# fgnt/padertorch

Measured on AMD Instinct MI355X. Metric: training frames/sec (PIT mask-est, 2-spk 8 kHz), higher is better.
Workload: dtype f32

## Files before the change

include/ptmi.h:

```cpp
#ifndef PTMI_H_
#define PTMI_H_

#include <stdint.h>

#ifdef __cplusplus
extern "C" {
#endif

#define PTMI_OK 0
#define PTMI_E_INVALID (-1)
#define PTMI_E_UNSUPPORTED (-2)

typedef void* ptmi_stream_t;

const char* ptmi_version(void);
const char* ptmi_error_string(int code);

typedef struct ptmi_stft_geom {
    int32_t size;
    int32_t shift;
    int32_t window_length;
    int32_t pad_left;
    int32_t pad_right;
    int32_t pad;
// ... 51 lines not shown


int ptmi_lstm_forward(float* gates, float* hy, float* c, const float* c0, const float* w_hh_pad, const int32_t* batch_sizes,
                      const int64_t* offsets, int32_t T, int32_t max_batch, int32_t H, int32_t KP,
                      int32_t ndir, ptmi_stream_t stream);

int ptmi_lstm_backward(const float* gates, const float* c, const float* c0, const float* dhy, const float* w_hh_t, float* dgates,
                       float* dc_state, const int32_t* batch_sizes, const int64_t* offsets, int32_t T,
                       int32_t max_batch, int32_t H, int32_t ndir, ptmi_stream_t stream);

int64_t ptmi_lstm_flags_elems(int32_t T, int32_t ndir, int32_t max_batch);
int64_t ptmi_lstm_scratch_elems(int32_t T, int32_t ndir, int32_t max_batch, int32_t H, int32_t backward);
int ptmi_lstm_weight_prep(const float* const* w_ih, const float* const* w_hh, const float* const* b_ih,
                          const float* const* b_hh, int32_t ndir, int32_t H, int32_t I, float* w_ih_cat, int32_t Ipad,
                          float* bias, float* w_pad, int32_t KP, float* w_t, uint32_t* amax, ptmi_stream_t stream);
int ptmi_lstm_set_error_sink(uint32_t* word);
int ptmi_lstm_split_enabled(void);
int32_t ptmi_lstm_handoff_cols(int32_t H, int32_t backward);
int32_t ptmi_lstm_backward_planes_ok(int32_t T, int32_t ndir, int32_t max_batch, int64_t rows, int32_t H);
int ptmi_lstm_forward_fills(int32_t T, int32_t ndir, int32_t max_batch, int32_t H);

int ptmi_lstm_forward_persistent(float* gates, float* hy, float* c, const float* c0, const float* w_hh_pad,
                                 const uint32_t* w_hh_amax, const int32_t* batch_sizes_dev, const int64_t* offsets_dev,
                                 const uint64_t* step_masks, uint32_t* flags, int32_t T, int32_t max_batch, int64_t rows,
                                 int32_t H, int32_t KP, int32_t ndir, int32_t prefilled, uint32_t* backward_scratch,
                                 ptmi_stream_t stream);

int ptmi_lstm_backward_persistent(const float* gates, const float* c, const float* c0, const float* dhy, const float* dc_n,
                                  const float* w_hh_t, float* dgates, uint16_t* dgates_t, const int32_t* batch_sizes_dev,
                                  const int64_t* offsets_dev, const uint64_t* step_masks, uint32_t* flags, float* dc_carry,
// ... 188 lines not shown
```

padertorch_amd/_lib.py:

```python
import ctypes
import os
import threading
from ctypes import c_char_p, c_double, c_float, c_int, c_int32, c_int64, c_void_p, POINTER
from pathlib import Path

import torch

_PKG = Path(__file__).resolve().parent
LIB_PATH = _PKG / 'libptmi.so'
if os.environ.get('PTMI_LIB'):
    LIB_PATH = Path(os.environ['PTMI_LIB'])


class StftGeom(ctypes.Structure):
    _fields_ = [('size', c_int32), ('shift', c_int32), ('window_length', c_int32),
                ('pad_left', c_int32), ('pad_right', c_int32), ('pad', c_int32)]


class NormGeom(ctypes.Structure):
    _fields_ = [('rank', c_int32), ('size', c_int64 * 5), ('stat_group_stride', c_int64 * 5),
                ('indep_stride', c_int64 * 5), ('batch_dim', c_int32), ('seq_dim', c_int32)]


_P = c_void_p
_G = POINTER(StftGeom)
_I64P = POINTER(c_int64)

SIGNATURES = {
    'ptmi_version': (c_char_p, []),
    'ptmi_error_string': (c_char_p, [c_int]),
    'ptmi_stft_num_frames': (c_int64, [_G, c_int64]),
    'ptmi_istft_num_samples': (c_int64, [_G, c_int64]),
    'ptmi_stft_forward': (c_int, [_P, c_int64, c_int64, c_int64, _P, _P, _P, _G, c_int64, c_int32,
                                  c_float, _P, _P]),
    'ptmi_istft_forward': (c_int, [_P, c_int64, c_int64, _P, _P, _P, _G, c_int32, c_float, c_int64,
                                   c_int64, c_int64, _P, _P]),
# ... 64 lines not shown
    'ptmi_dprnn_colsum': (c_int, [_P, c_int64, _P, _P, _P, c_int64, c_int32, _P]),
    'ptmi_dprnn_norm_residual_forward': (c_int, [_P, _P, _P, _P, _P, _P, _P, c_int64, c_int32, c_int32, c_int32, c_float, _P]),
    'ptmi_dprnn_norm_residual_backward': (c_int, [_P, _P, _P, _P, _P, _P, _P, _P, _P, c_int64, c_int32, c_int32, c_int32, _P]),
    'ptmi_dprnn_segment': (c_int, [_P, _I64P, _P, c_int64, c_int64, c_int32, c_int32, c_int32, c_int32, _P]),
    'ptmi_dprnn_overlap_add': (c_int, [_P, _I64P, _P, c_int64, c_int64, c_int32, c_int32, c_int32, c_int32, c_int32, _P]),
    'ptmi_lstm_forward': (c_int, [_P, _P, _P, _P, _P, _P, _P, c_int32, c_int32, c_int32, c_int32, c_int32, _P]),
    'ptmi_lstm_backward': (c_int, [_P, _P, _P, _P, _P, _P, _P, _P, _P, c_int32, c_int32, c_int32, c_int32, _P]),
    'ptmi_unit_norm_forward': (c_int, [_P, _P, _P, c_int64, c_int32, c_int32, c_float, c_void_p]),
    'ptmi_unit_norm_backward': (c_int, [_P, _P, _P, _P, c_int64, c_int32, c_int32, c_float, c_void_p]),
    'ptmi_lstm_flags_elems': (c_int64, [c_int32, c_int32, c_int32]),
    'ptmi_lstm_scratch_elems': (c_int64, [c_int32, c_int32, c_int32, c_int32, c_int32]),
    'ptmi_lstm_weight_prep': (c_int, [_P, _P, _P, _P, c_int32, c_int32, c_int32, _P, c_int32, _P, _P, c_int32, _P, _P, _P]),
    'ptmi_lstm_set_error_sink': (c_int, [_P]),
    'ptmi_lstm_split_enabled': (c_int, []),
    'ptmi_lstm_handoff_cols': (c_int32, [c_int32, c_int32]),
    'ptmi_lstm_forward_persistent': (c_int, [_P, _P, _P, _P, _P, _P, _P, _P, _P, _P, c_int32, c_int32, c_int64, c_int32, c_int32,
                                             c_int32, c_int32, _P, _P]),
    'ptmi_lstm_forward_fills': (c_int, [c_int32, c_int32, c_int32, c_int32]),
    'ptmi_lstm_backward_planes_ok': (c_int32, [c_int32, c_int32, c_int32, c_int64, c_int32]),
    'ptmi_lstm_backward_persistent': (c_int, [_P, _P, _P, _P, _P, _P, _P, _P, _P, _P, _P, _P, _P, c_int32, c_int32, c_int64, c_int32,
                                              c_int32, c_int32, c_int32, c_int32, _P]),
    'ptmi_absmax': (c_int, [_P, c_int64, c_int64, c_int64, _P, _P]),
    'ptmi_absmax_accumulate': (c_int, [_P, c_int64, c_int64, c_int64, _P, _P]),
    'ptmi_planes_elems': (c_int64, [c_int64, c_int64]),
    'ptmi_pack_planes_t': (c_int, [_P, c_int64, c_int64, c_int64, _P, _P, _P]),
    'ptmi_gemm_planes_workspace_elems': (c_int64, [c_int32, c_int32, c_int32, c_int32]),
    'ptmi_pack_planes_n': (c_int, [_P, c_int64, c_int64, c_int64, _P, _P, _P]),
    'ptmi_gemm_planes': (c_int, [_P, _P, _P, _P, _P, _P, c_int64, c_int32, c_int32, c_int32, c_int32, c_int32, c_int32, _P, _P]),
    'ptmi_gemm_planes_relu': (c_int, [_P, _P, _P, _P, _P, _P, c_int64, c_int32, c_int32, c_int32, c_int32, c_int32, _P, _P, c_int32, _P]),
    'ptmi_relu_backward_absmax': (c_int, [_P, _P, _P, c_int64, c_int64, c_int64, c_int64, c_int64, _P, c_int32, _P]),
# ... 184 lines not shown
```

padertorch_amd/csrc/gemm_planes.hip:

```cpp
#include <algorithm>

#include "common.h"

namespace ptmi {

typedef _Float16 h8 __attribute__((ext_vector_type(8)));
typedef __bf16 b8 __attribute__((ext_vector_type(8)));
typedef float f4 __attribute__((ext_vector_type(4)));

constexpr int PBM = 128, PBN = 128;
constexpr int FR = 64;

__device__ __forceinline__ float plane_scale(const unsigned* amax_bits) {
    if (!amax_bits) return 1.f;
    const unsigned e = (*amax_bits >> 23) & 0xffu;
    if (e == 0u || e == 0xffu) return 1.f;
    return __uint_as_float((unsigned)(127 + 13 + 127 - (int)e) << 23);
}

struct PlanesArgs {
    const uint4* A;
    const uint4* B;
    float* C;
    float* workspace;
    const unsigned* amax_a;
    const unsigned* amax_b;
    const float* bias;
    int M, N, KB;
    long long ldc;
    int accumulate;
    int kb_per_split;
    int tiles_m, tiles_n;
    float* C2 = nullptr;
// ... 503 lines not shown
        }
    } else {
        for (long long i = blockIdx.x * 256ll + threadIdx.x; i < n; i += (long long)gridDim.x * 256) {
            const long long r = i / cols, c = i - r * cols;
            m = max(m, __float_as_uint(x[r * ld + c]) & 0x7fffffffu);
        }
    }
#pragma unroll
    for (int o = 32; o > 0; o >>= 1) m = max(m, (unsigned)__shfl_xor((int)m, o));
    if ((threadIdx.x & 63) == 0) red[threadIdx.x >> 6] = m;
    __syncthreads();
    if (threadIdx.x == 0) {
        m = max(max(red[0], red[1]), max(red[2], red[3]));
        if (m >= 0x7f800000u) m = 0x7f7fffffu;
        atomicMax(out, m);
    }
}

template <bool BF16>
__device__ __forceinline__ void split_chunk(const float (&v)[8], uint4* hi_out, uint4* lo_out) {
    if (BF16) {
        b8 hi, lo;
#pragma unroll
        for (int e = 0; e < 8; ++e) {
            hi[e] = (__bf16)v[e];
            lo[e] = (__bf16)(v[e] - (float)hi[e]);
        }
        *hi_out = __builtin_bit_cast(uint4, hi);
        *lo_out = __builtin_bit_cast(uint4, lo);
    } else {
        h8 hi, lo;
#pragma unroll
        for (int e = 0; e < 8; ++e) {
            hi[e] = (_Float16)v[e];
            lo[e] = (_Float16)(v[e] - (float)hi[e]);
        }
        *hi_out = __builtin_bit_cast(uint4, hi);
        *lo_out = __builtin_bit_cast(uint4, lo);
    }
}

__global__ __launch_bounds__(256) void planes_reduce_kernel(const float* __restrict__ ws, int splits, float* __restrict__ C, long long ldc,
                                                            const float* __restrict__ bias, int M, int N, int accumulate,
                                                            float* __restrict__ C2 = nullptr, int m_split = 0, int relu = 0,
                                                            unsigned* __restrict__ amax_out = nullptr) {
    const long long total = (long long)M * N;
    unsigned mx = 0u;
    for (long long i = blockIdx.x * 256ll + threadIdx.x; i < total; i += (long long)gridDim.x * 256) {
        const int r = (int)(i / N), c = (int)(i - (long long)r * N);
        float sum = 0.f;
        for (int z = 0; z < splits; ++z) sum += ws[(long long)z * total + i];
        if (bias) sum += bias[c];
        if (relu) {
// ... 740 lines not shown
```

padertorch_amd/csrc/lstm_prep.hip:

```cpp
#include "common.h"

namespace ptmi {

constexpr int kIhPerWg = 16384;
constexpr int kStrip = 4;

struct PrepArgs {
    const float* w_ih[2];
    const float* w_hh[2];
    const float* b_ih[2];
    const float* b_hh[2];
    float* w_ih_cat;
    float* bias;
    float* w_pad;
    float* w_t;
    unsigned* amax;
    int ndir, G, I, Ipad, H, KP;
    int vec_ih;
    int blocks_ih;
    int tiles_g, strips_h;
};

__device__ __forceinline__ void publish_max(unsigned* word, float m, unsigned* red) {
    unsigned u = __float_as_uint(m);
// ... 136 lines not shown
    A.vec_ih = (I & 3) == 0 && Ipad == I;
    for (int d = 0; d < ndir; ++d) A.vec_ih = A.vec_ih && (reinterpret_cast<uintptr_t>(w_ih[d]) & 15) == 0;
    PTMI_RETURN_IF(reinterpret_cast<uintptr_t>(w_ih_cat) & 15, PTMI_E_INVALID);
    const long long total_ih = (long long)ndir * A.G * Ipad;
    A.blocks_ih = (int)((total_ih + kIhPerWg - 1) / kIhPerWg);
    A.tiles_g = (A.G + 31) / 32;
    A.strips_h = (KP + 32 * kStrip - 1) / (32 * kStrip);
    const int blocks_bias = (ndir * A.G + 255) / 256;
    hipStream_t st = static_cast<hipStream_t>(stream);
    hipError_t e = zero_words_async(amax, 2, st);
    if (e != hipSuccess) return (int)e;
    const unsigned grid = (unsigned)(A.blocks_ih + ndir * A.tiles_g * A.strips_h + blocks_bias);
    hipLaunchKernelGGL(lstm_weight_prep_kernel, dim3(grid), dim3(256), 0, st, A);
    return launch_status();
}
```

padertorch_amd/ops/gemm.py:

```python
import ctypes
import os
import threading
import weakref

import torch

from .. import _lib
from . import library

__all__ = ['mm', 'absmax', 'weight_absmax', 'UNIT_RANGE', 'PRODUCTS', 'ENABLED', 'usable']

ENABLED = True

PRODUCTS = 3

UNIT_RANGE = 'unit'

_WEIGHT_AMAX = {}


def _refs(params):
    return tuple(weakref.ref(p) for p in params)


# ... 100 lines not shown
    if len(cache) > limit:
        cache.clear()
    with torch.no_grad():
        v = make()
    cache[key] = (p._version, p.data_ptr(), v, _refs((p,)), _PREFETCHING[0])
    if form is not None:
        known = _KNOWN.get(id(p))
        if known is None or known[0]() is not p:
            if len(_KNOWN) > 256:
                _KNOWN.clear()
            known = _KNOWN[id(p)] = (weakref.ref(p), set())
        known[1].add(form)
    return v


def prefetch_known(device, everything=False):
    todo = []
    updated = _UPDATED.get(device)
    covered = updated[1] if updated is not None else {}
    for pid, (ref, forms) in list(_KNOWN.items()):
        q = ref()
        if q is None:
            del _KNOWN[pid]
        elif q.device == device and q.dim() == 2:
            e = covered.get(id(q))
            if everything or (e is not None and e[0]() is q and e[1] == q._version):
                todo.append((q, sorted(forms, key=str)))
    if not todo or _PREFETCHING[0] is not None:
        return
    ev = _PREFETCHING[0] = torch.cuda.Event()
    try:
        for q, forms in todo:
            for form in forms:
                if form == 'n':
                    weight_planes(q)
                elif form == 't':
                    weight_planes_t(q)
                else:
                    weight_planes_h(q, *form[1:])
    finally:
        _PREFETCHING[0] = None
        ev.record(torch.cuda.current_stream(device))


def weight_absmax(p):
    return _cached(_WEIGHT_AMAX, id(p), p, lambda: absmax(p.detach() if p.dim() == 2 else p.detach().reshape(-1, p.shape[-1])), 256)


def weights_absmax(params):
    params = tuple(params)
    if len(params) == 1:
        return weight_absmax(params[0])
    key = tuple(id(p) for p in params)
    sig = tuple((p._version, p.data_ptr()) for p in params)
    hit = _WEIGHT_AMAX.get(key)
    if hit is not None and hit[0] == sig and _same(hit[3], params):
        return hit[2]
# ... 187 lines not shown
```

padertorch_amd/ops/library.py:

```python
import ctypes
from typing import List, Optional, Tuple

import torch
from torch import Tensor

from .. import _lib

_LIBRARY = torch.library.Library('ptmi', 'DEF')


def _register(schema):
    name = schema.split('(', 1)[0].strip()

    def deco(fn):
        _LIBRARY.define(schema)
        _LIBRARY.impl(name, fn, 'CUDA')
        return getattr(torch.ops.ptmi, name)
    return deco


def _geom(g: List[int]):
    return _lib.StftGeom(*[int(v) for v in g])


# ... 539 lines not shown
@_register('lstm_weight_prep(Tensor[] w_ih, Tensor[] w_hh, Tensor[] b_ih, Tensor[] b_hh, int KP) -> '
           '(Tensor, Tensor, Tensor, Tensor, Tensor)')
def lstm_weight_prep(w_ih, w_hh, b_ih, b_hh, KP):
    ndir, (G, I), H = len(w_ih), w_ih[0].shape, w_hh[0].shape[1]
    dev = w_ih[0].device
    Ipad = (I + 3) // 4 * 4
    f32 = dict(dtype=torch.float32, device=dev)
    w_ih_cat, bias = torch.empty((ndir * G, Ipad), **f32), torch.empty(ndir * G, **f32)
    w_pad, w_t = torch.empty((ndir, G, KP), **f32), torch.empty((ndir, H, G), **f32)
    amax = torch.empty(2, dtype=torch.int32, device=dev)
    ptrs = [(ctypes.c_void_p * ndir)(*[t.data_ptr() for t in ts]) for ts in (w_ih, w_hh, b_ih, b_hh)]
    _lib.check(_lib.timed('lstm_weight_prep', _lib.load().ptmi_lstm_weight_prep, *ptrs, ndir, H, I, w_ih_cat.data_ptr(), Ipad,
                          bias.data_ptr(), w_pad.data_ptr(), KP, w_t.data_ptr(), amax.data_ptr(), _lib.stream(dev)),
               'ptmi_lstm_weight_prep')
    return w_ih_cat, bias, w_pad, w_t, amax


@_register('grad_norm(Tensor flat) -> Tensor')
def grad_norm(flat):
    lib = _lib.load()
    ws = torch.empty(int(lib.ptmi_grad_norm_workspace_elems()), dtype=torch.float64, device=flat.device)
    out = torch.empty((), dtype=torch.float32, device=flat.device)
    _lib.check(_lib.timed('grad_norm', lib.ptmi_grad_norm, flat.data_ptr(), flat.numel(), ws.data_ptr(), out.data_ptr(),
                          _lib.stream(flat.device)), 'ptmi_grad_norm')
    return out


@_register('adam_flat_(Tensor(a!) flat_grad, Tensor(b!) exp_avg, Tensor(c!) exp_avg_sq, Tensor segments, Tensor(d!)[] params, '
           'Tensor? norm, float max_norm, Tensor? found_inf, Tensor? finite, Tensor step, float lr, float beta1, float beta2, '
           'float eps, float weight_decay, bool zero_grad, Tensor? hyper=None) -> Tensor')
# ... 372 lines not shown
```

padertorch_amd/ops/lstm.py:

```python
import types

import torch
from torch.nn.utils.rnn import PackedSequence

from .. import _lib
from . import capture as _capture
from . import context as _context
from . import gemm as _gemm
from . import library
from . import lstm_forms as _forms
from . import watchdog as _watchdog
from . import wgrad as _wgrad
from .lstm_forms import begin_captured_step, end_captured_step
from .pack_meta import _PackMeta, _meta, pack_meta
from .watchdog import check_errors, error_count, error_word, errors_since_last_report, raise_timeout
from .wgrad import flush_pending as flush_pending_wgrad, gemm_keys_safe, sync_deferred, warm_side_stream, wgrad_key

__all__ = ['packed_lstm']


PERSISTENT = True
CHECK_PERSISTENT_ERRORS = False
DEFER_WGRAD = False
GRAD_READY_HOOK = None
# ... 578 lines not shown
    else:
        assert meta.rows == data.shape[0] and hx is None and not return_state and input_planes is None, 'row-slot batches: plain calls only'
        if not (PERSISTENT and _lib.load().ptmi_lstm_split_enabled()):
            raise NotImplementedError('row-slot batches need the persistent split recurrence kernels')
    sfx = ['', '_reverse'] if lstm.bidirectional else ['']
    ndir, H = len(sfx), lstm.hidden_size
    want_state = return_state or hx is not None
    if hx is not None:
        h_all, c_all = hx
        assert h_all.shape == c_all.shape == (lstm.num_layers * ndir, meta.max_batch, H), (h_all.shape, meta.max_batch)
    h_n, c_n = [], []
    h = data.contiguous()
    all_params = [tuple((getattr(lstm, f'weight_ih_l{layer}{s}'), getattr(lstm, f'weight_hh_l{layer}{s}'),
                         getattr(lstm, f'bias_ih_l{layer}{s}'), getattr(lstm, f'bias_hh_l{layer}{s}')) for s in sfx)
                  for layer in range(lstm.num_layers)]
    forked, pre0 = _forms.fork_preparation(all_params, data, H, oc.defer_wgrad, DX_FROM_HANDOFF)
    prev_handoff = None
    for layer in range(lstm.num_layers):
        params = all_params[layer]
        graph = torch.is_grad_enabled() and any(p.requires_grad for ps in params for p in ps)
        in_place = oc.defer_wgrad and all(p.requires_grad and p.is_leaf and p.grad is not None for ps in params for p in ps)
        forms = anchor = None
        if data.is_cuda and (not graph or in_place):
            forms = _forms.stacked_weights(params, _forms.kpad_of(H), DX_FROM_HANDOFF)
            if forms.ready is not None:
                torch.cuda.current_stream(data.device).wait_event(forms.ready)
            w_ih, bias, w_hh = forms.w_ih, forms.bias, forms.w_hh
            anchor = params[0][0] if graph else None
        else:
            w_ih = torch.cat([ps[0] for ps in params], 0)
            bias = torch.cat([ps[2] + ps[3] for ps in params], 0)
# ... 9 lines not shown
            hv, cv = h.view(meta.rows, ndir, H), c.view(meta.rows, ndir, H)
            h_n += [hv[meta.last_rows[d], d] for d in range(ndir)]
            c_n += [cv[meta.last_rows[d], d] for d in range(ndir)]
        else:
            out_handoff = {}
            if oc.grad_use_hook is not None and graph and in_place:
                oc.grad_use_hook([p for ps in params for p in ps])
            if layer == 0 and input_planes is not None and prev_handoff is None:
                prev_handoff = {'xplanes': input_planes}
            h = _LstmLayerFn.apply(h, w_ih, bias, w_hh, meta, None, None, params, layer > 0, anchor, forms, prev_handoff, out_handoff,
                                   layer + 1 == lstm.num_layers, oc)
            prev_handoff = out_handoff
        if lstm.dropout > 0 and training and layer + 1 < lstm.num_layers:
            h = torch.nn.functional.dropout(h, lstm.dropout, True)
            prev_handoff = None
    _forms.join_preparation(data.device, forked, pre0)
    if not (torch.is_grad_enabled() and h.requires_grad):
        check_errors()
    if prev_handoff and prev_handoff.get('planes') is not None:
        setattr(h, HANDOFF_ATTR, (h._version, prev_handoff['planes'], ndir, H))
    out = PackedSequence(h, packed.batch_sizes)
    if want_state:
        return out, (torch.stack(h_n), torch.stack(c_n))
    return out
```

padertorch_amd/ops/lstm_forms.py:

```python
import torch

from .. import _lib
from . import gemm as _gemm

_STACKED = {}
_PREP_STREAMS = {}
_EARLY_FORK = {}


def clear():
    _STACKED.clear()


def reset_step():
    _EARLY_FORK.clear()


def kpad_of(H):
    return (H + 15) // 16 * 16


def _prep_stream(device, first_layer=False):
    key = _lib.device_key(device) + (bool(first_layer),)
    if key not in _PREP_STREAMS:
        _PREP_STREAMS[key] = torch.cuda.Stream(device=device)
    return _PREP_STREAMS[key]


def begin_captured_step(device):
    from . import capture as _capture
    assert _capture.ACTIVE
    device = torch.device(device)
    pre, pre0 = _prep_stream(device), _prep_stream(device, True)
    pre.wait_stream(torch.cuda.current_stream(device))
    pre0.wait_stream(torch.cuda.current_stream(device))
    _EARLY_FORK[_lib.device_key(device)] = (pre, pre0)


def end_captured_step(device):
    device = torch.device(device)
    for side in _EARLY_FORK.pop(_lib.device_key(device), ()):
        torch.cuda.current_stream(device).wait_stream(side)


def _stacked_stale(params):
    flat = tuple(p for ps in params for p in ps)
    hit = _STACKED.get(tuple(id(p) for p in flat))
    return hit is None or hit[0] != tuple((p._version, p.data_ptr()) for p in flat) or not _gemm._same(hit[2], flat)


class _LazyPlanes:
# ... 70 lines not shown
    flat_ps = tuple(p for ps in params for p in ps)
    hit = _STACKED.get(key)
    if hit is not None and hit[0] == sig and _gemm._same(hit[2], flat_ps):
        return hit[1]
    if len(_STACKED) > 64:
        _STACKED.clear()
    with torch.no_grad():
        if params[0][0].is_cuda and all(p.dtype == torch.float32 and p.is_contiguous() for ps in params for p in ps):
            forms = _forms_kernel(params, KP, dx_from_handoff, stream)
        else:
            forms = _forms_torch(params, KP)
    _STACKED[key] = (sig, forms, _gemm._refs(flat_ps))
    return forms


def fork_preparation(all_params, data, H, defer_wgrad, dx_from_handoff):
    flat_params = [p for ps_ in all_params for ps in ps_ for p in ps]
    if not (data.is_cuda and any(_stacked_stale(ps_) for ps_ in all_params)
            and all(p.is_cuda and p.dtype == torch.float32 for p in flat_params)
            and (not (torch.is_grad_enabled() and any(p.requires_grad for p in flat_params))
                 or (defer_wgrad and all(p.requires_grad and p.is_leaf and p.grad is not None for p in flat_params)))):
        return None, None
    pre = _prep_stream(data.device)
    updated = _gemm.update_event(flat_params)
    from . import capture as _capture
    early = _EARLY_FORK.get(_lib.device_key(data.device)) if _capture.ACTIVE else None
    pre0 = early[1] if early else None
    early = bool(early)
    if early:
        pass
    elif updated is not None:
        pre.wait_event(updated)
    else:
        pre.wait_stream(torch.cuda.current_stream(data.device))
    for layer, ps_ in enumerate(all_params):
        if _stacked_stale(ps_) and (layer > 0 or pre0 is not None):
            stacked_weights(ps_, kpad_of(H), dx_from_handoff, stream=pre if layer > 0 else pre0)
    if updated is not None or early:
        with torch.cuda.stream(pre):
            _gemm.prefetch_known(data.device, everything=early)
    return pre, pre0


def join_preparation(device, forked, pre0):
    from . import capture as _capture
    if _capture.ACTIVE and forked is not None:
        torch.cuda.current_stream(device).wait_stream(forked)
        if pre0 is not None:
            torch.cuda.current_stream(device).wait_stream(pre0)
```

Baseline: 1.249 million.

## Batch per-step LSTM and dense weight form preparation into two table-driven kernels

Replaces the many per-layer weight-prep launches and the separate prefetch of dense GEMM planes with a precomputed job table. Two grouped kernels then run over all layers and dense weights: one for absmax and one that writes copies, transposes and fp16/bf16 split planes. The table is cached by parameter identity and pointers. The aim is to cut kernel launch count and host overhead on the preparation stream after each optimizer step. It adds a double-buffered absmax word scheme and drops the separate early-fork stream for layer 0.

```diff
diff --git a/include/ptmi.h b/include/ptmi.h
--- a/include/ptmi.h
+++ b/include/ptmi.h
@@ -89,6 +89,25 @@
 int ptmi_lstm_weight_prep(const float* const* w_ih, const float* const* w_hh, const float* const* b_ih,
                           const float* const* b_hh, int32_t ndir, int32_t H, int32_t I, float* w_ih_cat, int32_t Ipad,
                           float* bias, float* w_pad, int32_t KP, float* w_t, uint32_t* amax, ptmi_stream_t stream);
+typedef struct ptmi_forms_job {
+    const float* src;
+    const float* src2;
+    float* copy;
+    float* tr;
+    uint16_t* n_out;
+    uint16_t* t_out;
+    int32_t kind, rows, cols, ld;
+    int32_t amax_group, scale_group;
+    int32_t copy_ld, copy_cols, tr_ld;
+    int32_t n_rt0, n_kbs, n_kbo, n_kbn;
+    int32_t t_bf16, t_c0, t_climit, t_kbs, t_kbo, t_kbn;
+    int32_t src_aligned, copy_aligned, row_blocks, col_tiles, strips, wg_start, awg_start, awg_count, group_wgs;
+} ptmi_forms_job;
+int64_t ptmi_step_forms_plan(ptmi_forms_job* jobs, int32_t n_jobs, int32_t n_groups);
+int ptmi_step_forms_absmax(const ptmi_forms_job* jobs_dev, int32_t n_jobs, int64_t workgroups, uint32_t* words, int32_t n_groups,
+                           ptmi_stream_t stream);
+int ptmi_step_forms_write(const ptmi_forms_job* jobs_dev, int32_t n_jobs, int64_t workgroups, uint32_t* words, int32_t n_groups,
+                          ptmi_stream_t stream);
 int ptmi_lstm_set_error_sink(uint32_t* word);
 int ptmi_lstm_split_enabled(void);
 int32_t ptmi_lstm_handoff_cols(int32_t H, int32_t backward);
diff --git a/padertorch_amd/_lib.py b/padertorch_amd/_lib.py
--- a/padertorch_amd/_lib.py
+++ b/padertorch_amd/_lib.py
@@ -20,6 +20,13 @@
 class NormGeom(ctypes.Structure):
     _fields_ = [('rank', c_int32), ('size', c_int64 * 5), ('stat_group_stride', c_int64 * 5),
                 ('indep_stride', c_int64 * 5), ('batch_dim', c_int32), ('seq_dim', c_int32)]
+
+
+class FormsJob(ctypes.Structure):
+    _fields_ = ([(n, c_void_p) for n in ('src', 'src2', 'copy', 'tr', 'n_out', 't_out')]
+                + [(n, c_int32) for n in ('kind', 'rows', 'cols', 'ld', 'amax_group', 'scale_group', 'copy_ld', 'copy_cols', 'tr_ld',
+                                          'n_rt0', 'n_kbs', 'n_kbo', 'n_kbn', 't_bf16', 't_c0', 't_climit', 't_kbs', 't_kbo', 't_kbn',
+                                          'src_aligned', 'copy_aligned', 'row_blocks', 'col_tiles', 'strips', 'wg_start', 'awg_start', 'awg_count', 'group_wgs')])
 
 
 _P = c_void_p
@@ -114,6 +121,9 @@
     'ptmi_lstm_set_error_sink': (c_int, [_P]),
     'ptmi_lstm_split_enabled': (c_int, []),
     'ptmi_lstm_handoff_cols': (c_int32, [c_int32, c_int32]),
+    'ptmi_step_forms_plan': (c_int64, [POINTER(FormsJob), c_int32, c_int32]),
+    'ptmi_step_forms_absmax': (c_int, [_P, c_int32, c_int64, _P, c_int32, _P]),
+    'ptmi_step_forms_write': (c_int, [_P, c_int32, c_int64, _P, c_int32, _P]),
     'ptmi_lstm_forward_persistent': (c_int, [_P, _P, _P, _P, _P, _P, _P, _P, _P, _P, c_int32, c_int32, c_int64, c_int32, c_int32,
                                              c_int32, c_int32, _P, _P]),
     'ptmi_lstm_forward_fills': (c_int, [c_int32, c_int32, c_int32, c_int32]),
diff --git a/padertorch_amd/csrc/gemm_planes.hip b/padertorch_amd/csrc/gemm_planes.hip
--- a/padertorch_amd/csrc/gemm_planes.hip
+++ b/padertorch_amd/csrc/gemm_planes.hip
@@ -1,22 +1,11 @@
 #include <algorithm>
 
 #include "common.h"
+#include "planes.h"
 
 namespace ptmi {
 
-typedef _Float16 h8 __attribute__((ext_vector_type(8)));
-typedef __bf16 b8 __attribute__((ext_vector_type(8)));
-typedef float f4 __attribute__((ext_vector_type(4)));
-
 constexpr int PBM = 128, PBN = 128;
-constexpr int FR = 64;
-
-__device__ __forceinline__ float plane_scale(const unsigned* amax_bits) {
-    if (!amax_bits) return 1.f;
-    const unsigned e = (*amax_bits >> 23) & 0xffu;
-    if (e == 0u || e == 0xffu) return 1.f;
-    return __uint_as_float((unsigned)(127 + 13 + 127 - (int)e) << 23);
-}
 
 struct PlanesArgs {
     const uint4* A;
@@ -550,29 +539,6 @@
         m = max(max(red[0], red[1]), max(red[2], red[3]));
         if (m >= 0x7f800000u) m = 0x7f7fffffu;
         atomicMax(out, m);
-    }
-}
-
-template <bool BF16>
-__device__ __forceinline__ void split_chunk(const float (&v)[8], uint4* hi_out, uint4* lo_out) {
-    if (BF16) {
-        b8 hi, lo;
-#pragma unroll
-        for (int e = 0; e < 8; ++e) {
-            hi[e] = (__bf16)v[e];
-            lo[e] = (__bf16)(v[e] - (float)hi[e]);
-        }
-        *hi_out = __builtin_bit_cast(uint4, hi);
-        *lo_out = __builtin_bit_cast(uint4, lo);
-    } else {
-        h8 hi, lo;
-#pragma unroll
-        for (int e = 0; e < 8; ++e) {
-            hi[e] = (_Float16)v[e];
-            lo[e] = (_Float16)(v[e] - (float)hi[e]);
-        }
-        *hi_out = __builtin_bit_cast(uint4, hi);
-        *lo_out = __builtin_bit_cast(uint4, lo);
     }
 }
 
diff --git a/padertorch_amd/csrc/lstm_prep.hip b/padertorch_amd/csrc/lstm_prep.hip
--- a/padertorch_amd/csrc/lstm_prep.hip
+++ b/padertorch_amd/csrc/lstm_prep.hip
@@ -1,4 +1,7 @@
+#include <algorithm>
+
 #include "common.h"
+#include "planes.h"
 
 namespace ptmi {
 
@@ -174,3 +177,274 @@
     hipLaunchKernelGGL(lstm_weight_prep_kernel, dim3(grid), dim3(256), 0, st, A);
     return launch_status();
 }
+
+namespace ptmi {
+
+constexpr int kFormTiles = 4;
+constexpr int kFormPitch = 65;
+
+typedef ptmi_forms_job FormsJob;
+
+__device__ __forceinline__ int forms_find_job(const FormsJob* __restrict__ jobs, int n_jobs, int wg) {
+    int lo = 0, hi = n_jobs - 1;
+    while (lo < hi) {
+        const int mid = (lo + hi + 1) >> 1;
+        if (jobs[mid].wg_start <= wg) lo = mid; else hi = mid - 1;
+    }
+    return lo;
+}
+
+__device__ __forceinline__ void forms_load_tile(const float* __restrict__ src, int rows, int cols, int ld, bool aligned, int r0, int c0, f4 (&v)[2]) {
+    const int lx = threadIdx.x & 15, ly = threadIdx.x >> 4;
+    const int c = c0 + lx * 4;
+#pragma unroll
+    for (int p = 0; p < 2; ++p) {
+        const int r = r0 + ly + p * 16;
+        f4 z = {0.f, 0.f, 0.f, 0.f};
+        if (r < rows && c < cols) {
+            const float* q = src + (size_t)r * ld + c;
+            if (aligned && c + 4 <= cols) {
+                z = *reinterpret_cast<const f4*>(q);
+            } else {
+#pragma unroll
+                for (int e = 0; e < 4; ++e)
+                    if (c + e < cols) z[e] = q[e];
+            }
+        }
+        v[p] = z;
+    }
+}
+
+constexpr int kAmaxStrips = 2;
+
+__device__ __forceinline__ int forms_find_amax_job(const FormsJob* __restrict__ jobs, int n_jobs, int wg) {
+    int lo = 0, hi = n_jobs - 1;
+    while (lo < hi) {
+        const int mid = (lo + hi + 1) >> 1;
+        if (jobs[mid].awg_start <= wg) lo = mid; else hi = mid - 1;
+    }
+    return lo;
+}
+
+__global__ __launch_bounds__(256) void forms_absmax_kernel(const FormsJob* __restrict__ jobs, int n_jobs, unsigned* __restrict__ words, int n_groups) {
+    __shared__ unsigned red[4];
+    const int wg = blockIdx.x;
+    const FormsJob& J = jobs[forms_find_amax_job(jobs, n_jobs, wg)];
+    const int group = J.amax_group;
+    const int strips = J.strips;
+    const unsigned set = words[3 * n_groups] & 1u;
+    const float* src = J.src;
+    const int rows = J.rows, cols = J.cols, ld = J.ld;
+    const bool aligned = J.src_aligned != 0;
+    const int first = (wg - J.awg_start) * kAmaxStrips;
+    const int last = min(first + kAmaxStrips, ((rows + 31) >> 5) * strips);
+    unsigned m = 0u;
+    for (int local = first; local < last; ++local) {
+        const int rb = local / strips, cs = local - rb * strips;
+        f4 v[kFormTiles][2];
+#pragma unroll
+        for (int t = 0; t < kFormTiles; ++t) forms_load_tile(src, rows, cols, ld, aligned, rb * 32, (cs * kFormTiles + t) * 64, v[t]);
+#pragma unroll
+        for (int t = 0; t < kFormTiles; ++t)
+#pragma unroll
+            for (int p = 0; p < 2; ++p)
+#pragma unroll
+                for (int e = 0; e < 4; ++e) m = max(m, __float_as_uint(v[t][p][e]) & 0x7fffffffu);
+    }
+#pragma unroll
+    for (int o = 32; o > 0; o >>= 1) m = max(m, (unsigned)__shfl_xor((int)m, o));
+    if ((threadIdx.x & 63) == 0) red[threadIdx.x >> 6] = m;
+    __syncthreads();
+    if (threadIdx.x == 0) {
+        m = max(max(red[0], red[1]), max(red[2], red[3]));
+        if (m >= 0x7f800000u) m = 0x7f7fffffu;
+        unsigned* acc = words + (1 + set) * n_groups + group;
+        if (m > __hip_atomic_load(acc, __ATOMIC_RELAXED, __HIP_MEMORY_SCOPE_AGENT)) atomicMax(acc, m);
+    }
+    if (wg == 0) {
+        for (int g = threadIdx.x; g < n_groups; g += 256) words[(2 - set) * n_groups + g] = 0u;
+        if (threadIdx.x == 0) words[3 * n_groups + 1] = set;
+    }
+}
+
+__global__ __launch_bounds__(256) void forms_write_kernel(const FormsJob* __restrict__ jobs, int n_jobs, unsigned* __restrict__ words, int n_groups) {
+    __shared__ float tile[32 * kFormPitch];
+    const int wg = blockIdx.x, tid = threadIdx.x;
+    const FormsJob& J = jobs[forms_find_job(jobs, n_jobs, wg)];
+    const int local = wg - J.wg_start;
+    const unsigned* maxima = words + (1 + (words[3 * n_groups + 1] & 1u)) * n_groups;
+    if (wg == 0) {
+        for (int g = tid; g < n_groups; g += 256) words[g] = maxima[g];
+        if (tid == 0) words[3 * n_groups] = 1u - (words[3 * n_groups + 1] & 1u);
+    }
+    if (J.kind == 1) {
+#pragma unroll
+        for (int e = 0; e < 4; ++e) {
+            const int i = local * 1024 + e * 256 + tid;
+            if (i < J.cols) J.copy[i] = J.src[i] + J.src2[i];
+        }
+        return;
+    }
+    const int strips = J.strips;
+    const int rb = local / strips, cs = local - rb * strips;
+    const float* src = J.src;
+    const int rows = J.rows, cols = J.cols, ld = J.ld;
+    const bool aligned = J.src_aligned != 0;
+    const int ntiles = min(kFormTiles, J.col_tiles - cs * kFormTiles);
+    f4 v[kFormTiles][2];
+#pragma unroll
+    for (int t = 0; t < kFormTiles; ++t)
+        if (t < ntiles) forms_load_tile(src, rows, cols, ld, aligned, rb * 32, (cs * kFormTiles + t) * 64, v[t]);
+    const float s = J.scale_group >= 0 ? plane_scale(maxima + J.scale_group) : 1.f;
+    float* copy = J.copy;
+    float* tr = J.tr;
+    uint4* n_out = reinterpret_cast<uint4*>(J.n_out);
+    uint4* t_out = reinterpret_cast<uint4*>(J.t_out);
+    const int lx = tid & 15, ly = tid >> 4;
+    const int rows16 = (rows + 15) & ~15;
+#pragma unroll
+    for (int t = 0; t < kFormTiles; ++t) {
+        if (t >= ntiles) break;
+        const int ct = cs * kFormTiles + t;
+        if (t > 0) __syncthreads();
+#pragma unroll
+        for (int p = 0; p < 2; ++p) {
+#pragma unroll
+            for (int e = 0; e < 4; ++e) tile[(ly + p * 16) * kFormPitch + lx * 4 + e] = v[t][p][e];
+            if (copy) {
+                const int r = rb * 32 + ly + p * 16, c = ct * 64 + lx * 4;
+                if (r < rows && c < J.copy_cols) {
+                    float* q = copy + (size_t)r * J.copy_ld + c;
+                    if (J.copy_aligned && c + 4 <= J.copy_cols) {
+                        *reinterpret_cast<f4*>(q) = v[t][p];
+                    } else {
+#pragma unroll
+                        for (int e = 0; e < 4; ++e)
+                            if (c + e < J.copy_cols) q[e] = v[t][p][e];
+                    }
+                }
+            }
+        }
+        __syncthreads();
+        if (tr) {
+            const int tx = tid & 31, ty = tid >> 5;
+            const int r = rb * 32 + tx;
+#pragma unroll
+            for (int q = 0; q < 8; ++q) {
+                const int cl = ty + q * 8, c = ct * 64 + cl;
+                if (r < rows && c < cols) tr[(size_t)c * J.tr_ld + r] = tile[tx * kFormPitch + cl];
+            }
+        }
+        const int g = (tid >> 4) & 3, r16 = tid & 15;
+        if (n_out) {
+            const int rtl = tid >> 7, kbl = (tid >> 6) & 1;
+            const int rt = rb * 2 + rtl, kb = ct * 2 + kbl;
+            if (rt * 16 < rows16 && kb < J.n_kbn) {
+                float x[8];
+#pragma unroll
+                for (int e = 0; e < 8; ++e) x[e] = tile[(rtl * 16 + r16) * kFormPitch + kbl * 32 + g * 8 + e] * s;
+                uint4* o = n_out + (((size_t)(J.n_rt0 + rt) * J.n_kbs + J.n_kbo + kb) * 2) * FR + g * 16 + r16;
+                split_chunk<false>(x, o, o + FR);
+            }
+        }
+        if (t_out) {
+            const int cl = (tid >> 6) * 16 + r16, c = ct * 64 + cl;
+            if (c < J.t_climit && rb < J.t_kbn) {
+                const int cabs = J.t_c0 + c;
+                uint4* o = t_out + (((size_t)(cabs >> 4) * J.t_kbs + J.t_kbo + rb) * 2) * FR + g * 16 + (cabs & 15);
+                float x[8];
+                if (J.t_bf16) {
+#pragma unroll
+                    for (int e = 0; e < 8; ++e) x[e] = tile[(g * 8 + e) * kFormPitch + cl];
+                    split_chunk<true>(x, o, o + FR);
+                } else {
+#pragma unroll
+                    for (int e = 0; e < 8; ++e) x[e] = tile[(g * 8 + e) * kFormPitch + cl] * s;
+                    split_chunk<false>(x, o, o + FR);
+                }
+            }
+        }
+    }
+}
+
+}
+
+extern "C" {
+
+int64_t ptmi_step_forms_plan(ptmi_forms_job* jobs, int32_t n_jobs, int32_t n_groups) {
+    PTMI_RETURN_IF(!jobs || n_jobs < 1 || n_groups < 0, PTMI_E_INVALID);
+    long long total = 0, amax_total = 0;
+    for (int i = 0; i < n_jobs; ++i) {
+        ptmi_forms_job& J = jobs[i];
+        PTMI_RETURN_IF(!J.src || J.rows < 1 || J.cols < 1 || J.ld < J.cols, PTMI_E_INVALID);
+        PTMI_RETURN_IF(J.amax_group < -1 || J.amax_group >= n_groups || J.scale_group < -1 || J.scale_group >= n_groups, PTMI_E_INVALID);
+        J.src_aligned = (reinterpret_cast<uintptr_t>(J.src) & 15) == 0 && (J.ld & 3) == 0;
+        J.copy_aligned = 0;
+        J.group_wgs = 0;
+        J.wg_start = (int32_t)total;
+        J.awg_start = (int32_t)amax_total;
+        J.awg_count = 0;
+        if (J.kind == 1) {
+            PTMI_RETURN_IF(!J.src2 || !J.copy || J.rows != 1 || J.tr || J.n_out || J.t_out || J.amax_group >= 0, PTMI_E_INVALID);
+            J.row_blocks = 1;
+            J.col_tiles = J.strips = (J.cols + 1023) / 1024;
+            total += J.strips;
+            continue;
+        }
+        PTMI_RETURN_IF(J.kind != 0, PTMI_E_INVALID);
+        int row_blocks = (J.rows + 31) / 32, col_tiles = (J.cols + 63) / 64;
+        if (J.copy) {
+            PTMI_RETURN_IF(J.copy_cols < J.cols || J.copy_ld < J.copy_cols, PTMI_E_INVALID);
+            J.copy_aligned = (reinterpret_cast<uintptr_t>(J.copy) & 15) == 0 && (J.copy_ld & 3) == 0;
+            col_tiles = std::max(col_tiles, (J.copy_cols + 63) / 64);
+        }
+        PTMI_RETURN_IF(J.tr && J.tr_ld < J.rows, PTMI_E_INVALID);
+        if (J.n_out) {
+            PTMI_RETURN_IF((reinterpret_cast<uintptr_t>(J.n_out) & 15) || J.n_rt0 < 0 || J.n_kbo < 0 || J.n_kbn < (J.cols + 31) / 32 ||
+                               J.n_kbo + J.n_kbn > J.n_kbs,
+                           PTMI_E_INVALID);
+            col_tiles = std::max(col_tiles, (J.n_kbn + 1) / 2);
+        }
+        if (J.t_out) {
+            PTMI_RETURN_IF((reinterpret_cast<uintptr_t>(J.t_out) & 15) || J.t_c0 < 0 || J.t_kbo < 0 || J.t_kbn < (J.rows + 31) / 32 ||
+                               J.t_kbo + J.t_kbn > J.t_kbs || J.t_climit < J.cols,
+                           PTMI_E_INVALID);
+            row_blocks = std::max(row_blocks, J.t_kbn);
+            col_tiles = std::max(col_tiles, (J.t_climit + 63) / 64);
+        }
+        J.row_blocks = row_blocks;
+        J.col_tiles = col_tiles;
+        J.strips = (col_tiles + kFormTiles - 1) / kFormTiles;
+        total += (long long)row_blocks * J.strips;
+        PTMI_RETURN_IF(total >= (1ll << 30), PTMI_E_UNSUPPORTED);
+        if (J.amax_group >= 0) J.awg_count = (int32_t)(((long long)((J.rows + 31) / 32) * J.strips + kAmaxStrips - 1) / kAmaxStrips);
+        amax_total += J.awg_count;
+    }
+    for (int i = 0; i < n_jobs; ++i) {
+        if (jobs[i].kind != 0 || jobs[i].amax_group < 0) continue;
+        int n = 0;
+        for (int k = 0; k < n_jobs; ++k)
+            if (jobs[k].kind == 0 && jobs[k].amax_group == jobs[i].amax_group) n += jobs[k].awg_count;
+        jobs[i].group_wgs = n;
+    }
+    return total;
+}
+
+int ptmi_step_forms_absmax(const ptmi_forms_job* jobs_dev, int32_t n_jobs, int64_t workgroups, uint32_t* words, int32_t n_groups,
+                           ptmi_stream_t stream) {
+    PTMI_RETURN_IF(!jobs_dev || n_jobs < 1 || workgroups < 0 || workgroups >= (1ll << 30) || n_groups < 0 || (n_groups && !words), PTMI_E_INVALID);
+    if (n_groups == 0 || workgroups == 0) return PTMI_OK;
+    hipLaunchKernelGGL(forms_absmax_kernel, dim3((unsigned)workgroups), dim3(256), 0, static_cast<hipStream_t>(stream), jobs_dev, (int)n_jobs, words,
+                       (int)n_groups);
+    return launch_status();
+}
+
+int ptmi_step_forms_write(const ptmi_forms_job* jobs_dev, int32_t n_jobs, int64_t workgroups, uint32_t* words, int32_t n_groups,
+                          ptmi_stream_t stream) {
+    PTMI_RETURN_IF(!jobs_dev || n_jobs < 1 || workgroups < 1 || workgroups >= (1ll << 30) || n_groups < 0 || (n_groups && !words), PTMI_E_INVALID);
+    hipLaunchKernelGGL(forms_write_kernel, dim3((unsigned)workgroups), dim3(256), 0, static_cast<hipStream_t>(stream), jobs_dev, (int)n_jobs, words,
+                       (int)n_groups);
+    return launch_status();
+}
+
+}
diff --git a/padertorch_amd/csrc/planes.h b/padertorch_amd/csrc/planes.h
--- /dev/null
+++ b/padertorch_amd/csrc/planes.h
@@ -0,0 +1,42 @@
+#pragma once
+#include "common.h"
+
+namespace ptmi {
+
+typedef _Float16 h8 __attribute__((ext_vector_type(8)));
+typedef __bf16 b8 __attribute__((ext_vector_type(8)));
+typedef float f4 __attribute__((ext_vector_type(4)));
+
+constexpr int FR = 64;
+
+__device__ __forceinline__ float plane_scale(const unsigned* amax_bits) {
+    if (!amax_bits) return 1.f;
+    const unsigned e = (*amax_bits >> 23) & 0xffu;
+    if (e == 0u || e == 0xffu) return 1.f;
+    return __uint_as_float((unsigned)(127 + 13 + 127 - (int)e) << 23);
+}
+
+template <bool BF16>
+__device__ __forceinline__ void split_chunk(const float (&v)[8], uint4* hi_out, uint4* lo_out) {
+    if (BF16) {
+        b8 hi, lo;
+#pragma unroll
+        for (int e = 0; e < 8; ++e) {
+            hi[e] = (__bf16)v[e];
+            lo[e] = (__bf16)(v[e] - (float)hi[e]);
+        }
+        *hi_out = __builtin_bit_cast(uint4, hi);
+        *lo_out = __builtin_bit_cast(uint4, lo);
+    } else {
+        h8 hi, lo;
+#pragma unroll
+        for (int e = 0; e < 8; ++e) {
+            hi[e] = (_Float16)v[e];
+            lo[e] = (_Float16)(v[e] - (float)hi[e]);
+        }
+        *hi_out = __builtin_bit_cast(uint4, hi);
+        *lo_out = __builtin_bit_cast(uint4, lo);
+    }
+}
+
+}
diff --git a/padertorch_amd/ops/gemm.py b/padertorch_amd/ops/gemm.py
--- a/padertorch_amd/ops/gemm.py
+++ b/padertorch_amd/ops/gemm.py
@@ -138,7 +138,7 @@
     return v
 
 
-def prefetch_known(device, everything=False):
+def known_forms(device, everything=False):
     todo = []
     updated = _UPDATED.get(device)
     covered = updated[1] if updated is not None else {}
@@ -150,6 +150,11 @@
             e = covered.get(id(q))
             if everything or (e is not None and e[0]() is q and e[1] == q._version):
                 todo.append((q, sorted(forms, key=str)))
+    return todo
+
+
+def prefetch_known(device, everything=False):
+    todo = known_forms(device, everything)
     if not todo or _PREFETCHING[0] is not None:
         return
     ev = _PREFETCHING[0] = torch.cuda.Event()
@@ -165,6 +170,17 @@
     finally:
         _PREFETCHING[0] = None
         ev.record(torch.cuda.current_stream(device))
+
+
+def seed_known(p, amax, planes, event):
+    def enter(cache, key, value, limit):
+        if len(cache) > limit:
+            cache.clear()
+        cache[key] = (p._version, p.data_ptr(), value, _refs((p,)), event)
+    enter(_WEIGHT_AMAX, id(p), amax, 256)
+    for form, v in planes.items():
+        key = id(p) if form == 'n' else ('t', id(p)) if form == 't' else ('h', id(p), form[3])
+        enter(_WEIGHT_PLANES, key, (v, amax), 64)
 
 
 def weight_absmax(p):
diff --git a/padertorch_amd/ops/library.py b/padertorch_amd/ops/library.py
--- a/padertorch_amd/ops/library.py
+++ b/padertorch_amd/ops/library.py
@@ -577,6 +577,17 @@
                           bias.data_ptr(), w_pad.data_ptr(), KP, w_t.data_ptr(), amax.data_ptr(), _lib.stream(dev)),
                'ptmi_lstm_weight_prep')
     return w_ih_cat, bias, w_pad, w_t, amax
+
+
+@_register('step_forms_(Tensor table, int n_jobs, int amax_workgroups, int workgroups, Tensor(a!) words, int n_groups) -> ()')
+def step_forms_(table, n_jobs, amax_workgroups, workgroups, words, n_groups):
+    assert table.dtype == torch.uint8 and table.is_contiguous() and table.numel() == n_jobs * ctypes.sizeof(_lib.FormsJob)
+    assert words.dtype == torch.int32 and words.is_contiguous() and words.numel() == 3 * n_groups + 2
+    lib, st = _lib.load(), _lib.stream(table.device)
+    _lib.check(_lib.timed('step_forms_absmax', lib.ptmi_step_forms_absmax, table.data_ptr(), n_jobs, amax_workgroups, words.data_ptr(), n_groups,
+                          st), 'ptmi_step_forms_absmax')
+    _lib.check(_lib.timed('step_forms_write', lib.ptmi_step_forms_write, table.data_ptr(), n_jobs, workgroups, words.data_ptr(), n_groups, st),
+               'ptmi_step_forms_write')
 
 
 @_register('grad_norm(Tensor flat) -> Tensor')
diff --git a/padertorch_amd/ops/lstm.py b/padertorch_amd/ops/lstm.py
--- a/padertorch_amd/ops/lstm.py
+++ b/padertorch_amd/ops/lstm.py
@@ -616,7 +616,7 @@
     all_params = [tuple((getattr(lstm, f'weight_ih_l{layer}{s}'), getattr(lstm, f'weight_hh_l{layer}{s}'),
                          getattr(lstm, f'bias_ih_l{layer}{s}'), getattr(lstm, f'bias_hh_l{layer}{s}')) for s in sfx)
                   for layer in range(lstm.num_layers)]
-    forked, pre0 = _forms.fork_preparation(all_params, data, H, oc.defer_wgrad, DX_FROM_HANDOFF)
+    forked = _forms.fork_preparation(all_params, data, H, oc.defer_wgrad, DX_FROM_HANDOFF)
     prev_handoff = None
     for layer in range(lstm.num_layers):
         params = all_params[layer]
@@ -656,7 +656,7 @@
         if lstm.dropout > 0 and training and layer + 1 < lstm.num_layers:
             h = torch.nn.functional.dropout(h, lstm.dropout, True)
             prev_handoff = None
-    _forms.join_preparation(data.device, forked, pre0)
+    _forms.join_preparation(data.device, forked)
     if not (torch.is_grad_enabled() and h.requires_grad):
         check_errors()
     if prev_handoff and prev_handoff.get('planes') is not None:
diff --git a/padertorch_amd/ops/lstm_forms.py b/padertorch_amd/ops/lstm_forms.py
--- a/padertorch_amd/ops/lstm_forms.py
+++ b/padertorch_amd/ops/lstm_forms.py
@@ -1,3 +1,5 @@
+import weakref
+
 import torch
 
 from .. import _lib
@@ -6,6 +8,8 @@
 _STACKED = {}
 _PREP_STREAMS = {}
 _EARLY_FORK = {}
+_LAST = {}
+_TABLES = {}
 
 
 def clear():
@@ -14,14 +18,21 @@
 
 def reset_step():
     _EARLY_FORK.clear()
+    from . import capture as _capture
+    if not _capture.ACTIVE:
+        for refs, H, dx in list(_LAST.values()):
+            all_params = [[tuple(r() for r in ps) for ps in ps_] for ps_ in refs]
+            if all(p is not None and p.is_cuda for ps_ in all_params for ps in ps_ for p in ps):
+                device = all_params[0][0][0].device
+                _table_for(all_params, H, dx, _dense_forms(device, True))
 
 
 def kpad_of(H):
     return (H + 15) // 16 * 16
 
 
-def _prep_stream(device, first_layer=False):
-    key = _lib.device_key(device) + (bool(first_layer),)
+def _prep_stream(device):
+    key = _lib.device_key(device)
     if key not in _PREP_STREAMS:
         _PREP_STREAMS[key] = torch.cuda.Stream(device=device)
     return _PREP_STREAMS[key]
@@ -31,10 +42,9 @@
     from . import capture as _capture
     assert _capture.ACTIVE
     device = torch.device(device)
-    pre, pre0 = _prep_stream(device), _prep_stream(device, True)
+    pre = _prep_stream(device)
     pre.wait_stream(torch.cuda.current_stream(device))
-    pre0.wait_stream(torch.cuda.current_stream(device))
-    _EARLY_FORK[_lib.device_key(device)] = (pre, pre0)
+    _EARLY_FORK[_lib.device_key(device)] = (pre,)
 
 
 def end_captured_step(device):
@@ -135,37 +145,214 @@
     return forms
 
 
+class _StepTable:
+
+    @classmethod
+    def make(cls, all_params, KP, H, dx_from_handoff, dense):
+        lib = _lib.load()
+        dev = all_params[0][0][0].device
+        G, ndir = 4 * H, len(all_params[0])
+        planes_on = _gemm.planes_enabled()
+        cols_h = int(lib.ptmi_lstm_handoff_cols(H, 0)) if planes_on else 0
+        if H % 4 or KP < H:
+            return None
+        f32 = dict(dtype=torch.float32, device=dev)
+        ceil = lambda a, b: (a + b - 1) // b
+        jobs, layers = [], []
+        n_groups = 2 * len(all_params) + len(dense)
+
+        def job(**kw):
+            j = _lib.FormsJob(amax_group=-1, scale_group=-1)
+            for k, v in kw.items():
+                setattr(j, k, v)
+            jobs.append(j)
+
+        for li, ps_ in enumerate(all_params):
+            I = ps_[0][0].shape[1]
+            if any(ps[0].shape != (G, I) or ps[1].shape != (G, H) or ps[2].shape != (G,) or ps[3].shape != (G,) for ps in ps_):
+                return None
+            Ipad = (I + 3) // 4 * 4
+            hand = bool(cols_h) and I == ndir * H
+            cols_b = int(lib.ptmi_lstm_handoff_cols(H, 1)) if (planes_on and dx_from_handoff) else 0
+            dx = bool(cols_b) and I == ndir * H
+            if (hand and cols_h % 32) or (dx and (cols_b % 32 or cols_b < G)):
+                return None
+            cat, bias = torch.empty((ndir * G, Ipad), **f32), torch.empty(ndir * G, **f32)
+            w_pad, w_t = torch.empty((ndir, G, KP), **f32), torch.empty((ndir, H, G), **f32)
+            planes_h = planes_n = planes_dx = None
+            if hand:
+                planes_h = torch.empty(ndir * G // 16 * (ndir * cols_h // 32) * 1024, dtype=torch.float16, device=dev)
+            elif planes_on:
+                planes_n = torch.empty(int(lib.ptmi_planes_elems(ndir * G, I)), dtype=torch.float16, device=dev)
+            if dx:
+                planes_dx = torch.empty(ceil(I, 16) * (ndir * cols_b // 32) * 1024, dtype=torch.bfloat16, device=dev)
+            nseg, W = (ndir, H) if hand else (1, I)
+            for d, ps in enumerate(ps_):
+                for sg in range(nseg):
+                    kw = dict(src=ps[0].data_ptr() + 4 * sg * W, rows=G, cols=W, ld=I, amax_group=2 * li, scale_group=2 * li,
+                              copy=cat.data_ptr() + 4 * (d * G * Ipad + sg * W), copy_ld=Ipad, copy_cols=Ipad - sg * W if sg == nseg - 1 else W)
+                    if hand:
+                        kw.update(n_out=planes_h.data_ptr(), n_rt0=d * G // 16, n_kbs=ndir * cols_h // 32, n_kbo=sg * cols_h // 32,
+                                  n_kbn=cols_h // 32)
+                    elif planes_n is not None:
+                        kw.update(n_out=planes_n.data_ptr(), n_rt0=d * G // 16, n_kbs=ceil(I, 32), n_kbo=0, n_kbn=ceil(I, 32))
+                    if dx:
+                        kw.update(t_out=planes_dx.data_ptr(), t_bf16=1, t_c0=sg * W,
+                                  t_climit=ceil(I, 16) * 16 - sg * W if sg == nseg - 1 else W, t_kbs=ndir * cols_b // 32,
+                                  t_kbo=d * cols_b // 32, t_kbn=cols_b // 32)
+                    job(**kw)
+                job(src=ps[1].data_ptr(), rows=G, cols=H, ld=H, amax_group=2 * li + 1, copy=w_pad[d].data_ptr(), copy_ld=KP, copy_cols=KP,
+                    tr=w_t[d].data_ptr(), tr_ld=G)
+                job(kind=1, src=ps[2].data_ptr(), src2=ps[3].data_ptr(), rows=1, cols=G, ld=G, copy=bias.data_ptr() + 4 * d * G)
+            layers.append(dict(I=I, cat=cat, bias=bias, w_pad=w_pad, w_t=w_t, planes_h=planes_h, planes_n=planes_n, planes_dx=planes_dx,
+                               cols_h=cols_h if hand else 0, cols_b=cols_b if dx else 0))
+        dense_out = []
+        for di, (q, forms) in enumerate(dense):
+            group = 2 * len(all_params) + di
+            rows, cols = q.shape
+            out, counted = {}, False
+            if 'n' in forms or 't' in forms:
+                kw = dict(src=q.data_ptr(), rows=rows, cols=cols, ld=cols, amax_group=group, scale_group=group)
+                if 'n' in forms:
+                    out['n'] = torch.empty(int(lib.ptmi_planes_elems(rows, cols)), dtype=torch.float16, device=dev)
+                    kw.update(n_out=out['n'].data_ptr(), n_kbs=ceil(cols, 32), n_kbn=ceil(cols, 32))
+                if 't' in forms:
+                    out['t'] = torch.empty(int(lib.ptmi_planes_elems(cols, rows)), dtype=torch.float16, device=dev)
+                    kw.update(t_out=out['t'].data_ptr(), t_climit=ceil(cols, 16) * 16, t_kbs=ceil(rows, 32), t_kbn=ceil(rows, 32))
+                job(**kw)
+                counted = True
+            for form in forms:
+                if form in ('n', 't'):
+                    continue
+                _, nd, Hq, cq = form
+                if cq % 32 or cols != nd * Hq or cq < Hq:
+                    continue
+                out[form] = torch.empty(ceil(rows, 16) * (nd * cq // 32) * 1024, dtype=torch.float16, device=dev)
+                for sg in range(nd):
+                    job(src=q.data_ptr() + 4 * sg * Hq, rows=rows, cols=Hq, ld=cols, amax_group=-1 if counted else group, scale_group=group,
+                        n_out=out[form].data_ptr(), n_kbs=nd * cq // 32, n_kbo=sg * cq // 32, n_kbn=cq // 32)
+                counted = True
+            dense_out.append(out if counted else None)
+        arr = (_lib.FormsJob * len(jobs))(*jobs)
+        wgs = int(lib.ptmi_step_forms_plan(arr, len(jobs), n_groups))
+        if wgs < 0:
+            _lib.check(wgs, 'ptmi_step_forms_plan')
+        self = cls()
+        self.n_jobs, self.wgs, self.n_groups = len(jobs), wgs, n_groups
+        self.amax_wgs = arr[len(jobs) - 1].awg_start + arr[len(jobs) - 1].awg_count
+        import ctypes
+        self.table = torch.frombuffer(bytearray(ctypes.string_at(arr, ctypes.sizeof(arr))), dtype=torch.uint8).to(dev)
+        self.words = torch.zeros(3 * n_groups + 2, dtype=torch.int32, device=dev)
+        self.layers, self.dense_out = layers, dense_out
+        self.KP, self.H, self.ndir = KP, H, ndir
+        self.jobs = list(arr)
+        return self
+
+    def bytes_moved(self):
+        r16 = lambda n: (n + 15) // 16 * 16
+        amax = read = written = 0
+        for j in self.jobs:
+            if j.kind == 1:
+                read, written = read + 8 * j.cols, written + 4 * j.cols
+                continue
+            read += 4 * j.rows * j.cols
+            amax += 4 * j.rows * j.cols if j.amax_group >= 0 else 0
+            written += 4 * j.rows * j.copy_cols if j.copy else 0
+            written += 4 * j.rows * j.cols if j.tr else 0
+            written += r16(j.rows) * j.n_kbn * 32 * 4 if j.n_out else 0
+            written += j.t_climit * j.t_kbn * 32 * 4 if j.t_out else 0
+        return amax, read, written
+
+    def run(self, all_params, dense, stream):
+        with torch.cuda.stream(stream), torch.no_grad():
+            torch.ops.ptmi.step_forms_(self.table, self.n_jobs, self.amax_wgs, self.wgs, self.words, self.n_groups)
+            ready = torch.cuda.Event()
+            ready.record(stream)
+        H, ndir = self.H, self.ndir
+        if len(_STACKED) > 64:
+            _STACKED.clear()
+        for li, (ps_, L) in enumerate(zip(all_params, self.layers)):
+            I, amax = L['I'], self.words[2 * li:2 * li + 2]
+            w_ih = L['cat'][:, :I]
+            planes = planes_h = planes_dx = None
+            if L['planes_h'] is not None:
+                planes_h = ((L['planes_h'], amax[0:1]), L['cols_h'])
+                planes = planes_h[0] if L['cols_h'] == H else _LazyPlanes(w_ih, amax[0:1])
+            elif L['planes_n'] is not None:
+                planes = (L['planes_n'], amax[0:1])
+            if L['planes_dx'] is not None:
+                planes_dx = (L['planes_dx'], L['cols_b'])
+            forms = LayerForms(w_ih, L['bias'], L['w_pad'][:, :, :H], L['w_pad'], L['w_t'], L['cat'] if L['cat'].shape[1] != I else None,
+                               planes, planes_h, planes_dx)
+            forms.ready = ready
+            flat = tuple(p for ps in ps_ for p in ps)
+            _STACKED[tuple(id(p) for p in flat)] = (tuple((p._version, p.data_ptr()) for p in flat), forms, _gemm._refs(flat))
+            _gemm.seed_weights_absmax([ps[0] for ps in ps_], amax[0:1])
+            _gemm.seed_weights_absmax([ps[1] for ps in ps_], amax[1:2])
+        base = 2 * len(all_params)
+        for di, ((q, _), out) in enumerate(zip(dense, self.dense_out)):
+            if out is not None:
+                _gemm.seed_known(q, self.words[base + di:base + di + 1], out, ready)
+
+
+def _dense_forms(device, everything):
+    return [(q, f) for q, f in _gemm.known_forms(device, everything=everything) if q.dtype == torch.float32 and q.is_contiguous()]
+
+
+def _table_for(all_params, H, dx_from_handoff, dense):
+    flat = [p for ps_ in all_params for ps in ps_ for p in ps] + [q for q, _ in dense]
+    if not all(p.is_cuda and p.dtype == torch.float32 and p.is_contiguous() for p in flat):
+        return None
+    key = (tuple(id(p) for p in flat), tuple(tuple(f) for _, f in dense), bool(dx_from_handoff), _gemm.planes_enabled())
+    ptrs = tuple((p.data_ptr(), tuple(p.shape)) for p in flat)
+    hit = _TABLES.get(key)
+    if hit is not None and hit[0] == ptrs and _gemm._same(hit[2], flat):
+        return hit[1]
+    from . import capture as _capture
+    if _capture.ACTIVE:
+        return None
+    for k in [k for k, v in _TABLES.items() if any(r() is None for r in v[2])] + (list(_TABLES) if len(_TABLES) > 8 else []):
+        _TABLES.pop(k, None)
+    table = _StepTable.make(all_params, kpad_of(H), H, dx_from_handoff, dense)
+    _TABLES[key] = (ptrs, table, _gemm._refs(flat))
+    return table
+
+
 def fork_preparation(all_params, data, H, defer_wgrad, dx_from_handoff):
     flat_params = [p for ps_ in all_params for ps in ps_ for p in ps]
     if not (data.is_cuda and any(_stacked_stale(ps_) for ps_ in all_params)
             and all(p.is_cuda and p.dtype == torch.float32 for p in flat_params)
             and (not (torch.is_grad_enabled() and any(p.requires_grad for p in flat_params))
                  or (defer_wgrad and all(p.requires_grad and p.is_leaf and p.grad is not None for p in flat_params)))):
-        return None, None
+        return None
     pre = _prep_stream(data.device)
     updated = _gemm.update_event(flat_params)
     from . import capture as _capture
-    early = _EARLY_FORK.get(_lib.device_key(data.device)) if _capture.ACTIVE else None
-    pre0 = early[1] if early else None
-    early = bool(early)
+    early = bool(_EARLY_FORK.get(_lib.device_key(data.device))) if _capture.ACTIVE else False
     if early:
         pass
     elif updated is not None:
         pre.wait_event(updated)
     else:
         pre.wait_stream(torch.cuda.current_stream(data.device))
+    dense = _dense_forms(data.device, early) if (updated is not None or early) else []
+    if len(_LAST) > 8:
+        _LAST.clear()
+    _LAST[_lib.device_key(data.device)] = ([[tuple(weakref.ref(p) for p in ps) for ps in ps_] for ps_ in all_params], H, dx_from_handoff)
+    table = _table_for(all_params, H, dx_from_handoff, dense)
+    if table is not None:
+        table.run(all_params, dense, pre)
+        return pre
     for layer, ps_ in enumerate(all_params):
-        if _stacked_stale(ps_) and (layer > 0 or pre0 is not None):
-            stacked_weights(ps_, kpad_of(H), dx_from_handoff, stream=pre if layer > 0 else pre0)
+        if _stacked_stale(ps_) and layer > 0:
+            stacked_weights(ps_, kpad_of(H), dx_from_handoff, stream=pre)
     if updated is not None or early:
         with torch.cuda.stream(pre):
             _gemm.prefetch_known(data.device, everything=early)
-    return pre, pre0
-
-
-def join_preparation(device, forked, pre0):
+    return pre
+
+
+def join_preparation(device, forked):
     from . import capture as _capture
     if _capture.ACTIVE and forked is not None:
         torch.cuda.current_stream(device).wait_stream(forked)
-        if pre0 is not None:
-            torch.cuda.current_stream(device).wait_stream(pre0)
```

Result: no change. 1.246 million (-0.2%).
